# nickirk/pymes

Measured on AMD Instinct MI355X. Metric: ccsd_iteration_time, lower is better.
Workload: dtype f64

## Files before the change

### pymes_amd/csrc/kernels.hip

```cpp
#include <hip/hip_runtime.h>
#include <type_traits>

#include <algorithm>
#include <atomic>
#include <chrono>
#include <cmath>
#include <cstdio>
#include <cstdlib>
#include <cstring>
#include <mutex>
#include <stdexcept>
#include <string>
#include <vector>

#include "device_api.h"
#include "diis_small.h"

#define HIP_CHECK(expr)                                                                   \
    do {                                                                                  \
        hipError_t err__ = (expr);                                                        \
        if (err__ != hipSuccess)                                                          \
            throw std::runtime_error(std::string("HIP error: ") + hipGetErrorString(err__) + \
                                     " at " __FILE__ ":" + std::to_string(__LINE__));     \
    } while (0)
// ... 1476 lines not shown
                for (int j = 0; j < NN; ++j) acc[i][j] = fma(p.x[i][e], p.y[j][e], acc[i][j]);
    __shared__ double sh[4][MM * NN];
    const int lane = threadIdx.x & 63, w = threadIdx.x >> 6;
#pragma unroll
    for (int i = 0; i < MM; ++i)
#pragma unroll
        for (int j = 0; j < NN; ++j) {
            const double s = wave_sum(acc[i][j]);
            if (lane == 0) sh[w][i * NN + j] = s;
        }
    __syncthreads();
    if (threadIdx.x < MM * NN)
        partial[(long)blockIdx.x * (MM * NN) + threadIdx.x] =
            (sh[0][threadIdx.x] + sh[1][threadIdx.x]) + (sh[2][threadIdx.x] + sh[3][threadIdx.x]);
}
__global__ void __launch_bounds__(256) gram_stage2_kernel(const double* __restrict__ partial, int nblocks, int cnt,
                                                          double* __restrict__ out) {
    __shared__ double sh[4];
    const int idx = blockIdx.x;
    double s = 0.0;
    for (int b = threadIdx.x; b < nblocks; b += blockDim.x) s += partial[(long)b * cnt + idx];
    s = block_sum(s, sh);
    if (threadIdx.x == 0) out[idx] = s;
}

template <int MM, int NN>
struct LinMulti {
    const double* x[MM];
    double* y[NN];
    double c[MM][NN];
    double beta[NN];
};
template <int MM, int NN, int VEC>
__global__ void __launch_bounds__(256) lincomb_multi_kernel(const LinMulti<MM, NN> p, int n, long len) {
    typedef double vec_t __attribute__((ext_vector_type(VEC)));
    const long nvec = len / VEC;
    for (long e = blockIdx.x * 256L + threadIdx.x; e < nvec; e += (long)gridDim.x * 256L) {
        vec_t xv[MM], out[NN];
#pragma unroll
        for (int i = 0; i < MM; ++i) xv[i] = reinterpret_cast<const vec_t*>(p.x[i])[e];
#pragma unroll
        for (int j = 0; j < NN; ++j) {
            vec_t s = 0.0;
            if (j < n && p.beta[j] != 0.0) s = p.beta[j] * reinterpret_cast<const vec_t*>(p.y[j])[e];
            out[j] = s;
        }
#pragma unroll
        for (int i = 0; i < MM; ++i)
#pragma unroll
            for (int j = 0; j < NN; ++j) out[j] += p.c[i][j] * xv[i];
#pragma unroll
        for (int j = 0; j < NN; ++j)
            if (j < n) reinterpret_cast<vec_t*>(p.y[j])[e] = out[j];
    }
    if (VEC > 1 && blockIdx.x == 0 && threadIdx.x == 0)
        for (long e = nvec * VEC; e < len; ++e) {
            double xs[MM], out[NN];
#pragma unroll
            for (int i = 0; i < MM; ++i) xs[i] = p.x[i][e];
#pragma unroll
            for (int j = 0; j < NN; ++j) out[j] = (j < n && p.beta[j] != 0.0) ? p.beta[j] * p.y[j][e] : 0.0;
#pragma unroll
            for (int i = 0; i < MM; ++i)
#pragma unroll
                for (int j = 0; j < NN; ++j) out[j] += p.c[i][j] * xs[i];
#pragma unroll
            for (int j = 0; j < NN; ++j)
                if (j < n) p.y[j][e] = out[j];
        }
}

__global__ void cmul_kernel(const double* __restrict__ mr, const double* __restrict__ mi, const double* xr, const double* xi,
                            double* yr, double* yi, long n) {
    for (long e = blockIdx.x * (long)blockDim.x + threadIdx.x; e < n; e += (long)gridDim.x * blockDim.x) {
        const double a = xr[e], b = xi[e], c = mr[e], d = mi[e];
        yr[e] = c * a - d * b;
        yi[e] = c * b + d * a;
    }
}

__global__ void exchange_split_kernel(const double* __restrict__ u, double* __restrict__ us, double* __restrict__ w,
                                      double* __restrict__ dg, int no, int nv, long total) {
    const long o = no, v = nv;
    for (long e = blockIdx.x * (long)blockDim.x + threadIdx.x; e < total; e += (long)gridDim.x * blockDim.x) {
        const long j = e % o, i = (e / o) % o, b = (e / (o * o)) % v, a = e / (o * o * v);
        const double x = u[e], y = u[((b * v + a) * o + j) * o + i];
        const double ua = 0.5 * (x - y);
        us[e] = 0.5 * (x + y);
        w[e] = i > j ? ua : (i < j ? -ua : 0.0);
        if (i == j) dg[(a * v + b) * o + i] = ua;
    }
}
__global__ void sgn_ij_add_kernel(double* __restrict__ D, const double* __restrict__ R, int no, long total) {
    const long o = no;
    for (long e = blockIdx.x * (long)blockDim.x + threadIdx.x; e < total; e += (long)gridDim.x * blockDim.x) {
        const long j = e % o, i = (e / o) % o;
        if (i != j) D[e] += (i > j ? R[e] : -R[e]);
    }
}

struct EomDiagWs {
    long S1, Sa, Si, A2, a_, i_, IJ, AJ, AB, Z1, X1, total;
    __host__ __device__ EomDiagWs(long o, long v) {
        long p = 0;
        S1 = p; p += v * o;  Sa = p; p += v;  Si = p; p += o;  A2 = p; p += v * o;  a_ = p; p += v;  i_ = p; p += o;
        IJ = p; p += o * o;  AJ = p; p += v * o;  AB = p; p += v * v;  Z1 = p; p += v * o * o;  X1 = p; p += v * v * o;
        total = p;
    }
};
__global__ void __launch_bounds__(256) eom_diag_sums_kernel(const double* __restrict__ V, const double* __restrict__ T,
                                                            double* __restrict__ ws, int no, int nv) {
    __shared__ double sh[4];
    const long o = no, v = nv;
    const EomDiagWs w(o, v);
    auto Vx = [&](long k, long l, long c, long d) { return V[((k * o + l) * v + c) * v + d]; };
    auto Tx = [&](long a, long b, long i, long j) { return T[((a * v + b) * o + i) * o + j]; };
    const long e = blockIdx.x;
    const int t = threadIdx.x;
    double s = 0.0;
    if (e < w.Sa) {
        const long a = e / o, i = e % o;
        for (long x = t; x < o * v; x += 256) {
            const long j = x / v, b = x % v;
            s += (2.0 * Vx(j, i, b, a) - Vx(j, i, a, b)) * (2.0 * Tx(b, a, j, i) - Tx(a, b, j, i));
        }
    } else if (e < w.Si) {
        const long a = e - w.Sa;
        for (long x = t; x < o * o * v; x += 256) {
            const long j = x / (o * v), k = (x / v) % o, b = x % v;
            s += (2.0 * Vx(j, k, b, a) - Vx(j, k, a, b)) * Tx(a, b, j, k);
        }
    } else if (e < w.A2) {
        const long i = e - w.Si;
        for (long x = t; x < o * v * v; x += 256) {
            const long j = x / (v * v), c = (x / v) % v, b = x % v;
            s += Vx(j, i, c, b) * Tx(b, c, j, i);
        }
    } else if (e < w.a_) {
        const long a = (e - w.A2) / o, i = (e - w.A2) % o;
        for (long x = t; x < o * v; x += 256) {
            const long k = x / v, c = x % v;
            const double tca = Tx(c, a, k, i), tac = Tx(a, c, k, i);
            s += (2.0 * Vx(k, i, c, a) - 2.0 * Vx(k, i, a, c)) * tca + (Vx(k, i, a, c) - 2.0 * Vx(k, i, c, a)) * tac;
            double vb = 0.0;
            for (long b = 0; b < v; ++b) vb += Vx(k, i, c, b);
            s += vb * tac;
        }
    } else if (e < w.i_) {
        const long a = e - w.a_;
        for (long x = t; x < o * o * v; x += 256) {
            const long k = x / (o * v), l = (x / v) % o, c = x % v;
            s += Vx(k, l, c, a) * (Tx(a, c, k, l) - 2.0 * Tx(c, a, k, l));
        }
    } else if (e < w.IJ) {
        const long i = e - w.i_;
        for (long x = t; x < o * v * v; x += 256) {
            const long k = x / (v * v), c = (x / v) % v, d = x % v;
            s += (Vx(k, i, d, c) - 2.0 * Vx(k, i, c, d)) * Tx(c, d, k, i);
        }
    } else if (e < w.AJ) {
        const long i = (e - w.IJ) / o, j = (e - w.IJ) % o;
        for (long x = t; x < v * v; x += 256) {
            const long c = x / v, d = x % v;
            s += Vx(i, j, c, d) * Tx(c, d, i, j);
        }
    } else if (e < w.AB) {
        const long a = (e - w.AJ) / o, j = (e - w.AJ) % o;
        for (long x = t; x < o * v; x += 256) {
            const long k = x / v, c = x % v;
            s += Vx(k, j, a, c) * Tx(a, c, k, j);
        }
    } else if (e < w.Z1) {
        const long a = (e - w.AB) / v, b = (e - w.AB) % v;
        for (long x = t; x < o * o; x += 256) {
            const long k = x / o, l = x % o;
            s += Vx(k, l, a, b) * Tx(a, b, k, l);
        }
    } else if (e < w.X1) {
        const long r = e - w.Z1, a = r / (o * o), i = (r / o) % o, j = r % o;
        for (long x = t; x < o * v; x += 256) {
            const long k = x / v, c = x % v;
            s += Vx(k, j, a, c) * Tx(c, a, k, i);
        }
    } else {
        const long r = e - w.X1, a = r / (v * o), b = (r / o) % v, j = r % o;
        for (long k = t; k < o; k += 256) s += Vx(k, j, a, b) * Tx(a, b, k, j);
    }
    s = block_sum(s, sh);
    if (t == 0) ws[e] = s;
}
__global__ void eom_diag_singles_kernel(const double* __restrict__ ws, const double* __restrict__ dai, const double* __restrict__ iaai,
                                        const double* __restrict__ iaia, double* __restrict__ d1, int no, int nv) {
    const long o = no, v = nv;
    const EomDiagWs w(o, v);
    const long e = blockIdx.x * (long)blockDim.x + threadIdx.x;
    if (e >= v * o) return;
    const long a = e / o, i = e % o;
    d1[e] = dai[e] + 2.0 * iaai[e] - iaia[e] + ws[w.S1 + e] - ws[w.Sa + a] - ws[w.Si + i];
}
__global__ void __launch_bounds__(256) eom_diag_doubles_kernel(const double* __restrict__ V, const double* __restrict__ T,
                                                               const double* __restrict__ ws, const double* __restrict__ dai,
                                                               const double* __restrict__ iaai, const double* __restrict__ iaia,
                                                               const double* __restrict__ ijij, const double* __restrict__ abab,
                                                               double* __restrict__ d2, int no, int nv, long total) {
    const long o = no, v = nv;
    const EomDiagWs w(o, v);
    auto Vx = [&](long k, long l, long c, long d) { return V[((k * o + l) * v + c) * v + d]; };
    auto Tx = [&](long a, long b, long i, long j) { return T[((a * v + b) * o + i) * o + j]; };
    auto half = [&](long a, long b, long i, long j) {
        const long ai = a * o + i;
        double r = dai[ai] + iaai[ai] - 2.0 * iaia[ai] + ws[w.A2 + ai] + ws[w.a_ + a] + ws[w.i_ + i] -
                   2.0 * ws[w.X1 + (a * v + b) * o + j] - 2.0 * ws[w.IJ + i * o + j] + ws[w.Z1 + (a * o + i) * o + j] +
                   ws[w.AJ + a * o + j];
        double y = 0.0;
        for (long k = 0; k < o; ++k) y += Vx(k, i, a, b) * Tx(a, b, k, j);
        for (long c = 0; c < v; ++c) y += Vx(i, j, c, a) * Tx(c, b, i, j);
        return r + y;
    };
    for (long e = blockIdx.x * (long)blockDim.x + threadIdx.x; e < total; e += (long)gridDim.x * blockDim.x) {
        const long j = e % o, i = (e / o) % o, b = (e / (o * o)) % v, a = e / (o * o * v);
        d2[e] = half(a, b, i, j) + half(b, a, j, i) + ijij[i * o + j] + ws[w.IJ + i * o + j] + ws[w.AB + a * v + b] + abab[a * v + b];
    }
}
__global__ void cshift_inv_kernel(const double* __restrict__ d, double zr, double zi, double hr, double hi, double shift,
                                  double* __restrict__ mr, double* __restrict__ mi, long n) {
    for (long e = blockIdx.x * (long)blockDim.x + threadIdx.x; e < n; e += (long)gridDim.x * blockDim.x) {
        const double x = zr - hr * d[e] + shift, y = zi - hi * d[e];
        const double q = x * x + y * y;
        mr[e] = x / q;
        mi[e] = -y / q;
    }
}

struct TauK {
    double* tau; const double* t2; const double* t1;
    long total;
    int no, nv;
};
__device__ __forceinline__ void tau_body(const TauK& k, const unsigned vb, const unsigned vgrid) {
    double* __restrict__ tau = k.tau;
    const double* __restrict__ t2 = k.t2;
    const double* __restrict__ t1 = k.t1;
    const int no = k.no, nv = k.nv;
    const long total = k.total;
    for (long idx = vb * (long)blockDim.x + threadIdx.x; idx < total; idx += (long)vgrid * blockDim.x) {
        long r = idx;
        const int j = (int)(r % no); r /= no;
        const int i = (int)(r % no); r /= no;
        const int b = (int)(r % nv);
        const int a = (int)(r / nv);
        tau[idx] = t2[idx] + t1[a * no + i] * t1[b * no + j];
    }
}
__global__ void tau_kernel(const TauK k) { tau_body(k, blockIdx.x, gridDim.x); }

__device__ __forceinline__ void unrank_pair(long r, int& x, int& y) {
    long xx = (long)((sqrt(8.0 * (double)r + 1.0) - 1.0) * 0.5);
    while (xx * (xx + 1) / 2 > r) --xx;
    while ((xx + 1) * (xx + 2) / 2 <= r) ++xx;
    x = (int)xx;
    y = (int)(r - xx * (xx + 1) / 2);
}

__global__ void __launch_bounds__(256) ladder_pack_V_kernel(const double* __restrict__ V, double* __restrict__ Vp,
                                                            double* __restrict__ Vm, int nr, int nv, long rp0,
                                                            int nt, long ntp, long npp, long npm) {
    __shared__ double sA[32][33], sB[32][33];
    const long bid = blockIdx.x;
    const long row = bid / ntp;
    const long tp = bid - row * ntp;
    int a = 1, b = 0, tc, td;
    if (nr > 0) unrank_pair(rp0 + row, a, b);
    unrank_pair(tp, tc, td);
    const double* __restrict__ Vab = V + (nr > 0 ? (long)a * nr + b : rp0 + row) * nv * nv;
    const int tx = threadIdx.x & 31, ty = threadIdx.x >> 5;
    const int c0 = tc * 32, d0 = td * 32;
#pragma unroll
    for (int j = 0; j < 4; ++j) {
        const int y = ty + 8 * j;
        if (c0 + y < nv && d0 + tx < nv) sA[y][tx] = Vab[(long)(c0 + y) * nv + d0 + tx];
        if (d0 + y < nv && c0 + tx < nv) sB[y][tx] = Vab[(long)(d0 + y) * nv + c0 + tx];
    }
    __syncthreads();
#pragma unroll
    for (int j = 0; j < 4; ++j) {
        const int y = ty + 8 * j;
        const int c = c0 + y, d = d0 + tx;
        if (c < nv && d < nv && c >= d) {
            const double x1 = sA[y][tx], x2 = sB[tx][y];
            Vp[row * npp + (long)c * (c + 1) / 2 + d] = x1 + x2;
            if (c > d) Vm[row * npm + (long)c * (c - 1) / 2 + d] = (a > b) ? x1 - x2 : 0.0;
        }
    }
}

__global__ void ladder_dress_tfrag_kernel(const double* __restrict__ t1, double* __restrict__ tf, int no, int nv, int nk, long total) {
    const long e = blockIdx.x * (long)blockDim.x + threadIdx.x;
    if (e >= total) return;
    const int L = (int)(e & 63), kk = (int)((e >> 6) % nk), tile = (int)((e >> 6) / nk);
    const int a = 16 * tile + (L & 15), k = 4 * kk + (L >> 4);
    tf[e] = (a < nv && k < no) ? -t1[(long)a * no + k] : 0.0;
}

template <int NK>
__global__ void __launch_bounds__(64) ladder_dress_kernel(const double* __restrict__ V, const double* __restrict__ Pk,
                                                          const double* __restrict__ tf, double* __restrict__ W, int no,
                                                          int nv, long ld, long row0, long row1, double sgn, long ntp) {
    constexpr int TP = 16 * 16 + 16;
    __shared__ double turn[16 * TP];
    const int lane = threadIdx.x, g = lane >> 4, c = lane & 15;
    const long idx = blockIdx.x >> 3;
    const long cdb = (blockIdx.x & 7) + 8 * (idx / ntp), tp = idx % ntp;
    if (cdb * 16 >= ld) return;
    int ta_, tb_;
    unrank_pair(tp, ta_, tb_);
    const int a0 = ta_ * 16, b0 = tb_ * 16;
    const long tri0 = (long)a0 * (a0 + 1) / 2;
    if (tri0 + (long)15 * a0 + 120 + b0 + 15 < row0 || tri0 + b0 >= row1) return;
    double ta[NK], tb[NK];
#pragma unroll
    for (int kk = 0; kk < NK; ++kk) {
        ta[kk] = tf[((long)ta_ * NK + kk) * 64 + lane];
        tb[kk] = tf[((long)tb_ * NK + kk) * 64 + lane];
    }
    typedef unsigned v2u __attribute__((ext_vector_type(2)));
    constexpr unsigned kOff = 0x80000000u;
    const long col = cdb * 16 + c;
    const unsigned lo = (unsigned)(8 * ((long)g * ld + col));
    const unsigned lo_last = (unsigned)(8 * ((long)(min(4 * (NK - 1) + g, no - 1) - 4 * (NK - 1)) * ld + col));
    const unsigned ldb = (unsigned)(8 * ld);
    const __amdgpu_buffer_rsrc_t rPa = __builtin_amdgcn_make_buffer_rsrc(const_cast<double*>(Pk + (long)a0 * no * ld), 0, kOff, 0x00020000);
    const __amdgpu_buffer_rsrc_t rPb = __builtin_amdgcn_make_buffer_rsrc(const_cast<double*>(Pk + (long)b0 * no * ld), 0, kOff, 0x00020000);
    const __amdgpu_buffer_rsrc_t rV = __builtin_amdgcn_make_buffer_rsrc(const_cast<double*>(V + (tri0 - row0) * ld), 0, kOff, 0x00020000);
    const __amdgpu_buffer_rsrc_t rW = __builtin_amdgcn_make_buffer_rsrc(W + (tri0 - row0) * ld, 0, kOff, 0x00020000);
    unsigned vo[4];
#pragma unroll
    for (int r = 0; r < 4; ++r) {
        const long a = a0 + g + 4 * r;
        vo[r] = a < nv ? (unsigned)(8 * ((a * (a + 1) / 2 - tri0) * ld + col)) : kOff;
    }
    auto row_off = [&](int r, int x) {
        const int a = a0 + g + 4 * r;
        const long row = (long)a * (a + 1) / 2 + x;
        return (x <= a && row >= row0 && row < row1) ? vo[r] : kOff;
    };
    constexpr int PA = 1, NBP = 2 * (PA + 1), VA = 3, NBV = 2 * (VA + 1);
    double pf[NBP][NK], vin[NBV][4];
    auto fetch_p = [&](int n) {
        const int x0 = n < 16 ? a0 : b0, i = n < 16 ? n : n - 16;
        const unsigned so = (unsigned)(min(x0 + i, nv - 1) - x0) * (unsigned)no * ldb;
        const __amdgpu_buffer_rsrc_t rs = n < 16 ? rPa : rPb;
#pragma unroll
        for (int kk = 0; kk < NK - 1; ++kk)
            pf[n % NBP][kk] = __builtin_bit_cast(double, __builtin_amdgcn_raw_buffer_load_b64(rs, lo, so + 4u * kk * ldb, 0));
        pf[n % NBP][NK - 1] = __builtin_bit_cast(double, __builtin_amdgcn_raw_buffer_load_b64(rs, lo_last, so + 4u * (NK - 1) * ldb, 0));
    };
    auto fetch_v = [&](int n) {
        const int x = b0 + n - 16;
#pragma unroll
        for (int r = 0; r < 4; ++r)
            vin[n % NBV][r] = __builtin_bit_cast(double, __builtin_amdgcn_raw_buffer_load_b64(rV, row_off(r, x), (unsigned)x * ldb, 2));
    };
#pragma unroll
    for (int n = 0; n < 2 * PA; ++n) fetch_p(n);
#pragma unroll
    for (int p = 0; p < 8; ++p) {
        const int n0 = 2 * p, n1 = n0 + 1;
        fetch_p(n0 + 2 * PA);
        fetch_p(n1 + 2 * PA);
        if (n0 + 2 * VA >= 16) { fetch_v(n0 + 2 * VA); fetch_v(n1 + 2 * VA); }
        v4d acc0 = {0.0, 0.0, 0.0, 0.0}, acc1 = {0.0, 0.0, 0.0, 0.0};
#pragma unroll
        for (int kk = 0; kk < NK; ++kk) {
            acc0 = __builtin_amdgcn_mfma_f64_16x16x4f64(tb[kk], pf[n0 % NBP][kk], acc0, 0, 0, 0);
            acc1 = __builtin_amdgcn_mfma_f64_16x16x4f64(tb[kk], pf[n1 % NBP][kk], acc1, 0, 0, 0);
        }
#pragma unroll
        for (int rb = 0; rb < 4; ++rb) {
            turn[n0 * TP + (g + 4 * rb) * 16 + c] = acc0[rb];
            turn[n1 * TP + (g + 4 * rb) * 16 + c] = acc1[rb];
        }
    }
    __builtin_amdgcn_fence(__ATOMIC_SEQ_CST, "wavefront");
    __builtin_amdgcn_wave_barrier();
    const double s2 = sgn > 0.0 ? -1.0 : 1.0;
#pragma unroll
    for (int p = 0; p < 8; ++p) {
        const int b = 2 * p, n0 = 16 + b, n1 = n0 + 1;
        if (n0 + 2 * PA < 32) { fetch_p(n0 + 2 * PA); fetch_p(n1 + 2 * PA); }
        if (n0 + 2 * VA < 32) { fetch_v(n0 + 2 * VA); fetch_v(n1 + 2 * VA); }
        v4d acc0, acc1;
#pragma unroll
        for (int r = 0; r < 4; ++r) {
            acc0[r] = fma(s2, turn[(g + 4 * r) * TP + b * 16 + c], vin[n0 % NBV][r]);
            acc1[r] = fma(s2, turn[(g + 4 * r) * TP + (b + 1) * 16 + c], vin[n1 % NBV][r]);
        }
#pragma unroll
        for (int kk = 0; kk < NK; ++kk) {
            acc0 = __builtin_amdgcn_mfma_f64_16x16x4f64(ta[kk], pf[n0 % NBP][kk], acc0, 0, 0, 0);
            acc1 = __builtin_amdgcn_mfma_f64_16x16x4f64(ta[kk], pf[n1 % NBP][kk], acc1, 0, 0, 0);
        }
#pragma unroll
        for (int h = 0; h < 2; ++h) {
            const int bb = b0 + b + h;
#pragma unroll
            for (int r = 0; r < 4; ++r) {
                const double val = (sgn > 0.0 && a0 + g + 4 * r == bb) ? 0.0 : (double)(h ? acc1[r] : acc0[r]);
                __builtin_amdgcn_raw_buffer_store_b64(__builtin_bit_cast(v2u, val), rW, row_off(r, bb), (unsigned)bb * ldb, 2);
            }
        }
    }
}

struct PackTK {
    const double* T; const double* t1; double* Sp; double* Am;
    long ldp, ldm, rp0;
    int no, nv, flags;
};
__device__ __forceinline__ void ladder_pack_T_body(const PackTK& k, const unsigned vb) {
    const double* __restrict__ T = k.T;
    const double* __restrict__ t1 = k.t1;
    double* __restrict__ Sp = k.Sp;
    double* __restrict__ Am = k.Am;
    const int no = k.no, nv = k.nv, flags = k.flags;
    const long ldp = k.ldp, ldm = k.ldm;
    const long row = k.rp0 + vb;
    int c, d;
    unrank_pair(row, c, d);
    const bool row_half = flags & dev::PACK_ROW_HALF, prow = flags & dev::PACK_AM_PROWS,
               col_half = flags & dev::PACK_COL_HALF, pcol = flags & dev::PACK_AM_PCOLS;
    const long o2 = (long)no * no;
    const double* __restrict__ T1 = T ? T + ((long)c * nv + d) * o2 : nullptr;
    const double* __restrict__ T2 = T ? T + ((long)d * nv + c) * o2 : nullptr;
    const double fr = (c == d && row_half) ? 0.25 : 0.5;
    const long mrow = prow ? row : (long)c * (c - 1) / 2 + d;
    const bool has_m = prow || c > d;
    if (threadIdx.x == 0) {
        const long opp = (long)no * (no + 1) / 2, mcols = pcol ? opp : opp - no;
        if (ldp > opp) Sp[row * ldp + opp] = 0.0;
        if (has_m && ldm > mcols) Am[mrow * ldm + mcols] = 0.0;
    }
    for (int e = threadIdx.x; e < o2; e += blockDim.x) {
        const int i = e / no, j = e - i * no;
        if (i < j) continue;
        double x1 = 0.0, x2 = 0.0;
        if (T) { x1 = T1[e]; x2 = T2[e]; }
        if (t1) {
            x1 += t1[(long)c * no + i] * t1[(long)d * no + j];
            x2 += t1[(long)d * no + i] * t1[(long)c * no + j];
        }
        Sp[row * ldp + (long)i * (i + 1) / 2 + j] = ((i == j && col_half) ? 0.5 * fr : fr) * (x1 + x2);
        if (has_m && (pcol || i > j)) {
            const long mcol = pcol ? (long)i * (i + 1) / 2 + j : (long)i * (i - 1) / 2 + j;
            Am[mrow * ldm + mcol] = (c > d && i > j) ? 0.5 * (x1 - x2) : 0.0;
        }
    }
}
__global__ void ladder_pack_T_kernel(const PackTK k) { ladder_pack_T_body(k, blockIdx.x); }

struct UnpackK {
    const double* L; double* R;
    double beta;
    long total;
    int no, nv;
};
__device__ __forceinline__ void ladder_unpack_body(const UnpackK& k, const unsigned vb, const unsigned vgrid) {
    const double* __restrict__ L = k.L;
    double* __restrict__ R = k.R;
    const double beta = k.beta;
    const int no = k.no, nv = k.nv;
    const long total = k.total;
    const long opp = (long)no * (no + 1) / 2, ld = (long)no * no;
    for (long idx = vb * (long)blockDim.x + threadIdx.x; idx < total; idx += (long)vgrid * blockDim.x) {
        long r = idx;
        const int j = (int)(r % no); r /= no;
        const int i = (int)(r % no); r /= no;
        const int b = (int)(r % nv);
        const int a = (int)(r / nv);
        const int ah = max(a, b), al = min(a, b), ih = max(i, j), il = min(i, j);
        const double* __restrict__ row = L + ((long)ah * (ah + 1) / 2 + al) * ld;
        double v = row[(long)ih * (ih + 1) / 2 + il];
        if (a != b && i != j) {
            const double x = row[opp + (long)ih * (ih - 1) / 2 + il];
            v += ((a > b) == (i > j)) ? x : -x;
        }
        R[idx] = (beta != 0.0) ? beta * R[idx] + v : v;
    }
}
__global__ void ladder_unpack_kernel(const UnpackK k) { ladder_unpack_body(k, blockIdx.x, gridDim.x); }

struct RingOpK {
    const double* Wd; const double* Ud; double* M; double* N1;
    double a1, a2;
    int no, nv;
};
__device__ __forceinline__ void ring_operands_body(const RingOpK& q, const unsigned vb) {
    const double* __restrict__ Wd = q.Wd;
    const double* __restrict__ Ud = q.Ud;
    double* __restrict__ M = q.M;
    double* __restrict__ N1 = q.N1;
    const double a1 = q.a1, a2 = q.a2;
    const int no = q.no, nv = q.nv;
    extern __shared__ double tile[];
    constexpr int CT = 32;
    const int k = vb / nv, b = vb - k * nv;
    const long ov = (long)no * nv;
    const double* __restrict__ wd = Wd + ((long)k * nv + b) * ((long)nv * no);
    const double* __restrict__ ud = Ud + ((long)k * nv + b) * ((long)no * nv);
    const long col = (long)b * no;
    for (int c0 = 0; c0 < nv; c0 += CT) {
        const int nc = min(CT, nv - c0);
        for (int e = threadIdx.x; e < no * CT; e += blockDim.x) {
            const int j = e / CT, cc = e - j * CT;
            if (cc < nc) tile[j * (CT + 1) + cc] = ud[(long)j * nv + c0 + cc];
        }
        __syncthreads();
        for (int e = threadIdx.x; e < nc * no; e += blockDim.x) {
            const int cc = e / no, j = e - cc * no;
            const double u = tile[j * (CT + 1) + cc];
            const double w = wd[(long)(c0 + cc) * no + j];
            const long off = ((long)(c0 + cc) * no + k) * ov + col + j;
            N1[off] = -u;
            M[off] = a1 * w - a2 * u;
        }
        __syncthreads();
    }
}
__global__ void __launch_bounds__(256) ring_operands_kernel(const RingOpK q) { ring_operands_body(q, blockIdx.x); }

struct LayoutsK {
    const double* T; double* Td; double* Tx; double* Ttd;
    double ca, cb;
    int no, nv;
};
template <bool RESIDUAL>
__device__ __forceinline__ void t2_layouts_body(const LayoutsK& k, const unsigned vb) {
    const double* __restrict__ T = k.T;
    double* __restrict__ Td = k.Td;
    double* __restrict__ Tx = k.Tx;
    double* __restrict__ Ttd = k.Ttd;
    const int no = k.no, nv = k.nv;
    const double ca = k.ca, cb = k.cb;
    extern __shared__ double tile[];
    const int a = vb / nv, b = vb - a * nv;
    const long o2 = (long)no * no, ov = (long)no * nv;
    const double* __restrict__ Tab = T + ((long)a * nv + b) * o2;
    const double* __restrict__ Tba = T + ((long)b * nv + a) * o2;
    const long base = (long)a * no * ov + (long)b * no;
    for (int e = threadIdx.x; e < o2; e += blockDim.x) {
        const int i = e / no, j = e - i * no;
        const double x = Tab[e];
        tile[i * (no + 1) + j] = x;
        const long off = base + (long)i * ov + j;
        if (Td) Td[off] = x;
        Ttd[off] = RESIDUAL ? 2.0 * x - Tba[e] : ca * x + cb * Tba[e];
    }
    __syncthreads();
    for (int e = threadIdx.x; e < o2; e += blockDim.x) {
        const int j = e / no, i = e - j * no;
        Tx[base + (long)j * ov + i] = tile[i * (no + 1) + j];
    }
}
template <bool RESIDUAL>
__global__ void __launch_bounds__(256) t2_layouts_kernel(const LayoutsK k) { t2_layouts_body<RESIDUAL>(k, blockIdx.x); }

struct AssembleK {
    const double* V; const double* L; const double* N; const double* D; const double* X; double* R;
    double xd;
    int no, nv;
};
__device__ __forceinline__ void residual_assemble_body(const AssembleK& k, const unsigned vb) {
    const double* V = k.V;
    const double* __restrict__ L = k.L;
    const double* __restrict__ N = k.N;
    const double* __restrict__ D = k.D;
    const double* __restrict__ X = k.X;
    double* R = k.R;
    const int no = k.no, nv = k.nv;
    const double xd = k.xd;
    extern __shared__ double S[];
    int a, b;
    unrank_pair(vb, a, b);
    const int p = no + 1;
    const long o2 = (long)no * no, ov = (long)no * nv, opp = (long)no * (no + 1) / 2;
    const long ab = ((long)a * nv + b) * o2, ba = ((long)b * nv + a) * o2;
    const long tab = (long)a * no * ov + (long)b * no, tba = (long)b * no * ov + (long)a * no;
    for (int e = threadIdx.x; e < o2; e += blockDim.x) {
        const int i = e / no, j = e - i * no;
        double v = N[ab + e] + D[tab + (long)i * ov + j] + X[tba + (long)i * ov + j];
        if (xd != 0.0) v += xd * X[tab + (long)i * ov + j];
        S[i * p + j] = v;
    }
    __syncthreads();
    for (int e = threadIdx.x; e < o2; e += blockDim.x) {
        const int j = e / no, i = e - j * no;
        double v = N[ba + e] + D[tba + (long)j * ov + i] + X[tab + (long)j * ov + i];
        if (xd != 0.0) v += xd * X[tba + (long)j * ov + i];
        S[i * p + j] += v;
    }
    __syncthreads();
    const double* __restrict__ row = L ? L + ((long)a * (a + 1) / 2 + b) * o2 : nullptr;
    for (int e = threadIdx.x; e < o2; e += blockDim.x) {
        const int i = e / no, j = e - i * no;
        const int ih = max(i, j), il = min(i, j);
        double ls = 0.0, la = 0.0;
        if (row) {
            ls = row[(long)ih * (ih + 1) / 2 + il];
            if (a != b && i != j) la = row[opp + (long)ih * (ih - 1) / 2 + il];
        }
        const double sgn = i > j ? 1.0 : -1.0;
        R[ab + e] = (V ? V[ab + e] : 0.0) + ls + sgn * la + S[i * p + j];
        if (a != b) R[ba + e] = (V ? V[ba + e] : 0.0) + ls - sgn * la + S[j * p + i];
    }
}
__global__ void __launch_bounds__(256) residual_assemble_kernel(const AssembleK k) { residual_assemble_body(k, blockIdx.x); }

__global__ void __launch_bounds__(256) energy_norms_pairs_kernel(const double* __restrict__ f, const double* __restrict__ t1,
                                                                 const double* __restrict__ tc, const double* __restrict__ Edir,
                                                                 const double* __restrict__ Eex, const double* __restrict__ dtc,
                                                                 int no, int nv, long r0, long npairs, int with_t1,
                                                                 double* __restrict__ partial) {
    __shared__ double sh[4];
    double s1 = 0.0, s2 = 0.0, s3 = 0.0, s4 = 0.0, s0 = 0.0, s5 = 0.0;
    const long o2 = (long)no * no;
    for (long tile = blockIdx.x; tile < 2 * npairs; tile += gridDim.x) {
        int a, b;
        unrank_pair(r0 + (tile >> 1), a, b);
        if (tile & 1) {
            if (a == b) continue;
            const int x = a; a = b; b = x;
        }
        const double* __restrict__ x = tc + tile * o2;
        const double* __restrict__ d = dtc ? dtc + tile * o2 : nullptr;
        const double* __restrict__ ed = Edir + ((long)a * nv + b) * o2;
        const double* __restrict__ ex = Eex + ((long)a * nv + b) * o2;
        for (int e = threadIdx.x; e < o2; e += blockDim.x) {
            const double v = x[e];
            double tau = v;
            if (t1) {
                const int i = e / no, j = e - i * no;
                tau += t1[a * no + i] * t1[b * no + j];
            }
            s1 += tau * ed[e];
            s2 += tau * ex[e];
            s3 += v * v;
            if (d) s4 += d[e] * d[e];
        }
    }
    if (with_t1 && t1 && f) {
        const long n = no + nv, ov = (long)no * nv;
        for (long e = blockIdx.x * (long)blockDim.x + threadIdx.x; e < ov; e += (long)gridDim.x * blockDim.x) {
            const long a = e / no, i = e - a * no;
            const double y = t1[e];
            s0 += f[i * n + no + a] * y;
            s5 += y * y;
        }
    }
    const double q0 = block_sum(s0, sh), q1 = block_sum(s1, sh), q2 = block_sum(s2, sh), q3 = block_sum(s3, sh),
                 q4 = block_sum(s4, sh), q5 = block_sum(s5, sh);
    if (threadIdx.x == 0) {
        partial[0 * kDotBlocks + blockIdx.x] = q0;
        partial[1 * kDotBlocks + blockIdx.x] = q1;
        partial[2 * kDotBlocks + blockIdx.x] = q2;
        partial[3 * kDotBlocks + blockIdx.x] = q3;
        partial[4 * kDotBlocks + blockIdx.x] = q4;
        partial[5 * kDotBlocks + blockIdx.x] = q5;
    }
}

__global__ void __launch_bounds__(256) pairs_pack_kernel(const double* __restrict__ full, double* __restrict__ Xc,
                                                         int no, int nv, long r0) {
    int a, b;
    unrank_pair(r0 + blockIdx.x, a, b);
    const long o2 = (long)no * no;
    const double* __restrict__ ab = full + ((long)a * nv + b) * o2;
    const double* __restrict__ ba = full + ((long)b * nv + a) * o2;
    double* __restrict__ out = Xc + (long)blockIdx.x * 2 * o2;
    for (int e = threadIdx.x; e < o2; e += blockDim.x) {
        out[e] = ab[e];
        out[o2 + e] = (a != b) ? ba[e] : 0.0;
    }
}
__global__ void __launch_bounds__(256) pairs_unpack_kernel(const double* __restrict__ Xc, double* __restrict__ full,
                                                           int no, int nv, long r0) {
    int a, b;
    unrank_pair(r0 + blockIdx.x, a, b);
    const long o2 = (long)no * no;
    const double* __restrict__ in = Xc + (long)blockIdx.x * 2 * o2;
    double* __restrict__ ab = full + ((long)a * nv + b) * o2;
    double* __restrict__ ba = full + ((long)b * nv + a) * o2;
    for (int e = threadIdx.x; e < o2; e += blockDim.x) {
        ab[e] = in[e];
        if (a != b) ba[e] = in[o2 + e];
    }
}
__global__ void __launch_bounds__(256) cc_update_pairs_kernel(double* __restrict__ tc, double* __restrict__ dtc,
                                                              const double* __restrict__ rc, const double* __restrict__ eo,
                                                              const double* __restrict__ ev, double shift, double delta,
                                                              int no, long r0) {
    int a, b;
    unrank_pair(r0 + blockIdx.x, a, b);
    const long o2 = (long)no * no, base = (long)blockIdx.x * 2 * o2;
    const double eab = ev[a] + ev[b];
    for (int e = threadIdx.x; e < 2 * o2; e += blockDim.x) {
        const int t = e >= o2 ? e - (int)o2 : e;
        const int i = t / no, j = t - i * no;
        const double x = rc[base + e] * (1.0 / (eo[i] + eo[j] - eab + shift));
        dtc[base + e] = x;
        tc[base + e] += delta * x;
    }
}
__global__ void __launch_bounds__(256) residual_assemble_pairs_kernel(const double* __restrict__ V, const double* __restrict__ L,
                                                                      const double* __restrict__ Np, const double* __restrict__ D,
                                                                      const double* __restrict__ X, double* __restrict__ Rc,
// ... 3084 lines not shown
```

Baseline: 0.1634.

## Split ladder dress kernel into interior and edge tile paths with V preloaded

Splits the ladder dressing kernel into a templated tile routine with a fast interior path that drops per-element bounds and row-range predicates, used when the tile is off-diagonal and fully inside the row window. The edge path skips whole MFMA pairs whose output rows fall outside the window. It also reorders the computation so V is loaded as the initial accumulator of the first MFMA stage, with the sign folded into tb, instead of added after the transposed turn. This is meant to cut address and predicate ALU work and wasted MFMAs on boundary tiles, at the cost of more code size and register pressure from two instantiations.

```diff
diff --git a/pymes_amd/csrc/kernels.hip b/pymes_amd/csrc/kernels.hip
--- a/pymes_amd/csrc/kernels.hip
+++ b/pymes_amd/csrc/kernels.hip
@@ -1802,114 +1802,165 @@
     tf[e] = (a < nv && k < no) ? -t1[(long)a * no + k] : 0.0;
 }
 
+typedef unsigned v2u_dress __attribute__((ext_vector_type(2)));
+
+template <int NK, bool EDGE>
+__device__ __forceinline__ void ladder_dress_tile(const double* __restrict__ V, const double* __restrict__ Pk,
+                                                  const double* __restrict__ tf, double* __restrict__ W, double* turn,
+                                                  int no, int nv, long ld, long row0, long row1, double sgn,
+                                                  int ta_, int tb_, long cdb) {
+    constexpr int TP = 16 * 16 + 16;
+    constexpr unsigned kOff = 0x80000000u;
+    const int lane = threadIdx.x, g = lane >> 4, c = lane & 15;
+    const int a0 = ta_ * 16, b0 = tb_ * 16;
+    const long tri0 = (long)a0 * (a0 + 1) / 2;
+    double ta[NK], tb[NK];
+#pragma unroll
+    for (int kk = 0; kk < NK; ++kk) {
+        ta[kk] = tf[((long)ta_ * NK + kk) * 64 + lane];
+        tb[kk] = tf[((long)tb_ * NK + kk) * 64 + lane];
+    }
+    if (sgn > 0.0) {
+#pragma unroll
+        for (int kk = 0; kk < NK; ++kk) tb[kk] = -tb[kk];
+    }
+    const long col = cdb * 16 + c;
+    const unsigned ldb = (unsigned)(8 * ld);
+    const unsigned lo = (unsigned)(8 * ((long)g * ld + col));
+    unsigned lk[NK];
+#pragma unroll
+    for (int kk = 0; kk < NK - 1; ++kk) lk[kk] = lo + 4u * kk * ldb;
+    lk[NK - 1] = (unsigned)(8 * ((long)min(4 * (NK - 1) + g, no - 1) * ld + col));
+    const __amdgpu_buffer_rsrc_t rPa = __builtin_amdgcn_make_buffer_rsrc(const_cast<double*>(Pk + (long)a0 * no * ld), 0, kOff, 0x00020000);
+    const __amdgpu_buffer_rsrc_t rPb = __builtin_amdgcn_make_buffer_rsrc(const_cast<double*>(Pk + (long)b0 * no * ld), 0, kOff, 0x00020000);
+    const __amdgpu_buffer_rsrc_t rV = __builtin_amdgcn_make_buffer_rsrc(const_cast<double*>(V + (tri0 - row0) * ld), 0, kOff, 0x00020000);
+    const __amdgpu_buffer_rsrc_t rW = __builtin_amdgcn_make_buffer_rsrc(W + (tri0 - row0) * ld, 0, kOff, 0x00020000);
+    unsigned vo[4];
+    int pr[4];
+#pragma unroll
+    for (int r = 0; r < 4; ++r) {
+        const int a = a0 + g + 4 * r;
+        pr[r] = (a - a0) * a0 + (a - a0) * (a - a0 + 1) / 2;
+        vo[r] = (!EDGE || a < nv) ? (unsigned)(8 * ((long)pr[r] * ld + col)) : kOff;
+    }
+    unsigned vl[4];
+#pragma unroll
+    for (int r = 0; r < 4; ++r) vl[r] = lo + 4u * r * ldb;
+    const int rlo = (int)max(-1L, min(row0 - tri0, 1L << 30)), rhi = (int)max(-1L, min(row1 - tri0, 1L << 30));
+    const unsigned span = (unsigned)max(0, rhi - rlo);
+    constexpr int PA = 1, NBP = 2 * (PA + 1), VA = 2, NBV = 2 * (VA + 1);
+    double pf[NBP][NK], vin[NBV][4];
+    auto fetch_p = [&](int n) {
+        const int x0 = n < 16 ? a0 : b0, i = n < 16 ? n : n - 16;
+        const unsigned so = (unsigned)(min(x0 + i, nv - 1) - x0) * (unsigned)no * ldb;
+        const __amdgpu_buffer_rsrc_t rs = n < 16 ? rPa : rPb;
+#pragma unroll
+        for (int kk = 0; kk < NK; ++kk)
+            pf[n % NBP][kk] = __builtin_bit_cast(double, __builtin_amdgcn_raw_buffer_load_b64(rs, lk[kk], so, 0));
+    };
+    auto fetch_v = [&](int n) {
+        const int a = a0 + n;
+        const unsigned so = ((unsigned)(n * a0 + b0) + (unsigned)(n * (n + 1) / 2)) * ldb;
+#pragma unroll
+        for (int r = 0; r < 4; ++r) {
+            unsigned off = vl[r];
+            if (EDGE) {
+                const int b = b0 + g + 4 * r, rel = n * a0 + n * (n + 1) / 2 + b;
+                if (!(a < nv && b <= a && (unsigned)(rel - rlo) < span)) off = kOff;
+            }
+            vin[n % NBV][r] = __builtin_bit_cast(double, __builtin_amdgcn_raw_buffer_load_b64(rV, off, so, 2));
+        }
+    };
+    auto live_a = [&](int n) {
+        const int a = a0 + n;
+        if (a >= nv || b0 > a) return false;
+        const int lo = n * a0 + n * (n + 1) / 2 + b0, hi = lo + min(15, a - b0);
+        return lo < rhi && hi >= rlo;
+    };
+    auto live_b = [&](int j) {
+        const int bb = b0 + j, d0 = max(a0, bb) - a0, d1 = min(a0 + 15, nv - 1) - a0;
+        if (d0 > d1) return false;
+        const int lo = d0 * a0 + d0 * (d0 + 1) / 2 + bb, hi = d1 * a0 + d1 * (d1 + 1) / 2 + bb;
+        return lo < rhi && hi >= rlo;
+    };
+#pragma unroll
+    for (int n = 0; n < 2 * PA; ++n) fetch_p(n);
+#pragma unroll
+    for (int n = 0; n < 2 * VA; ++n) fetch_v(n);
+#pragma unroll
+    for (int p = 0; p < 8; ++p) {
+        const int n0 = 2 * p, n1 = n0 + 1;
+        fetch_p(n0 + 2 * PA);
+        fetch_p(n1 + 2 * PA);
+        if (n0 + 2 * VA < 16) { fetch_v(n0 + 2 * VA); fetch_v(n1 + 2 * VA); }
+        if (EDGE && !live_a(n0) && !live_a(n1)) continue;
+        v4d acc0, acc1;
+#pragma unroll
+        for (int r = 0; r < 4; ++r) { acc0[r] = vin[n0 % NBV][r]; acc1[r] = vin[n1 % NBV][r]; }
+#pragma unroll
+        for (int kk = 0; kk < NK; ++kk) {
+            acc0 = __builtin_amdgcn_mfma_f64_16x16x4f64(tb[kk], pf[n0 % NBP][kk], acc0, 0, 0, 0);
+            acc1 = __builtin_amdgcn_mfma_f64_16x16x4f64(tb[kk], pf[n1 % NBP][kk], acc1, 0, 0, 0);
+        }
+#pragma unroll
+        for (int rb = 0; rb < 4; ++rb) {
+            turn[n0 * TP + (g + 4 * rb) * 16 + c] = acc0[rb];
+            turn[n1 * TP + (g + 4 * rb) * 16 + c] = acc1[rb];
+        }
+    }
+    __builtin_amdgcn_fence(__ATOMIC_SEQ_CST, "wavefront");
+    __builtin_amdgcn_wave_barrier();
+#pragma unroll
+    for (int p = 0; p < 8; ++p) {
+        const int b = 2 * p, n0 = 16 + b, n1 = n0 + 1;
+        if (n0 + 2 * PA < 32) { fetch_p(n0 + 2 * PA); fetch_p(n1 + 2 * PA); }
+        if (EDGE && !live_b(b) && !live_b(b + 1)) continue;
+        v4d acc0, acc1;
+#pragma unroll
+        for (int r = 0; r < 4; ++r) {
+            acc0[r] = turn[(g + 4 * r) * TP + b * 16 + c];
+            acc1[r] = turn[(g + 4 * r) * TP + (b + 1) * 16 + c];
+        }
+#pragma unroll
+        for (int kk = 0; kk < NK; ++kk) {
+            acc0 = __builtin_amdgcn_mfma_f64_16x16x4f64(ta[kk], pf[n0 % NBP][kk], acc0, 0, 0, 0);
+            acc1 = __builtin_amdgcn_mfma_f64_16x16x4f64(ta[kk], pf[n1 % NBP][kk], acc1, 0, 0, 0);
+        }
+#pragma unroll
+        for (int h = 0; h < 2; ++h) {
+            const int bb = b0 + b + h;
+#pragma unroll
+            for (int r = 0; r < 4; ++r) {
+                double val = h ? acc1[r] : acc0[r];
+                unsigned off = vo[r];
+                if (EDGE) {
+                    const int a = a0 + g + 4 * r;
+                    if (!(bb <= a && (unsigned)(pr[r] + bb - rlo) < span)) off = kOff;
+                    if (sgn > 0.0 && a == bb) val = 0.0;
+                }
+                __builtin_amdgcn_raw_buffer_store_b64(__builtin_bit_cast(v2u_dress, val), rW, off, (unsigned)bb * ldb, 2);
+            }
+        }
+    }
+}
+
 template <int NK>
 __global__ void __launch_bounds__(64) ladder_dress_kernel(const double* __restrict__ V, const double* __restrict__ Pk,
                                                           const double* __restrict__ tf, double* __restrict__ W, int no,
                                                           int nv, long ld, long row0, long row1, double sgn, long ntp) {
-    constexpr int TP = 16 * 16 + 16;
-    __shared__ double turn[16 * TP];
-    const int lane = threadIdx.x, g = lane >> 4, c = lane & 15;
+    __shared__ double turn[16 * (16 * 16 + 16)];
     const long idx = blockIdx.x >> 3;
     const long cdb = (blockIdx.x & 7) + 8 * (idx / ntp), tp = idx % ntp;
     if (cdb * 16 >= ld) return;
     int ta_, tb_;
     unrank_pair(tp, ta_, tb_);
     const int a0 = ta_ * 16, b0 = tb_ * 16;
-    const long tri0 = (long)a0 * (a0 + 1) / 2;
-    if (tri0 + (long)15 * a0 + 120 + b0 + 15 < row0 || tri0 + b0 >= row1) return;
-    double ta[NK], tb[NK];
-#pragma unroll
-    for (int kk = 0; kk < NK; ++kk) {
-        ta[kk] = tf[((long)ta_ * NK + kk) * 64 + lane];
-        tb[kk] = tf[((long)tb_ * NK + kk) * 64 + lane];
-    }
-    typedef unsigned v2u __attribute__((ext_vector_type(2)));
-    constexpr unsigned kOff = 0x80000000u;
-    const long col = cdb * 16 + c;
-    const unsigned lo = (unsigned)(8 * ((long)g * ld + col));
-    const unsigned lo_last = (unsigned)(8 * ((long)(min(4 * (NK - 1) + g, no - 1) - 4 * (NK - 1)) * ld + col));
-    const unsigned ldb = (unsigned)(8 * ld);
-    const __amdgpu_buffer_rsrc_t rPa = __builtin_amdgcn_make_buffer_rsrc(const_cast<double*>(Pk + (long)a0 * no * ld), 0, kOff, 0x00020000);
-    const __amdgpu_buffer_rsrc_t rPb = __builtin_amdgcn_make_buffer_rsrc(const_cast<double*>(Pk + (long)b0 * no * ld), 0, kOff, 0x00020000);
-    const __amdgpu_buffer_rsrc_t rV = __builtin_amdgcn_make_buffer_rsrc(const_cast<double*>(V + (tri0 - row0) * ld), 0, kOff, 0x00020000);
-    const __amdgpu_buffer_rsrc_t rW = __builtin_amdgcn_make_buffer_rsrc(W + (tri0 - row0) * ld, 0, kOff, 0x00020000);
-    unsigned vo[4];
-#pragma unroll
-    for (int r = 0; r < 4; ++r) {
-        const long a = a0 + g + 4 * r;
-        vo[r] = a < nv ? (unsigned)(8 * ((a * (a + 1) / 2 - tri0) * ld + col)) : kOff;
-    }
-    auto row_off = [&](int r, int x) {
-        const int a = a0 + g + 4 * r;
-        const long row = (long)a * (a + 1) / 2 + x;
-        return (x <= a && row >= row0 && row < row1) ? vo[r] : kOff;
-    };
-    constexpr int PA = 1, NBP = 2 * (PA + 1), VA = 3, NBV = 2 * (VA + 1);
-    double pf[NBP][NK], vin[NBV][4];
-    auto fetch_p = [&](int n) {
-        const int x0 = n < 16 ? a0 : b0, i = n < 16 ? n : n - 16;
-        const unsigned so = (unsigned)(min(x0 + i, nv - 1) - x0) * (unsigned)no * ldb;
-        const __amdgpu_buffer_rsrc_t rs = n < 16 ? rPa : rPb;
-#pragma unroll
-        for (int kk = 0; kk < NK - 1; ++kk)
-            pf[n % NBP][kk] = __builtin_bit_cast(double, __builtin_amdgcn_raw_buffer_load_b64(rs, lo, so + 4u * kk * ldb, 0));
-        pf[n % NBP][NK - 1] = __builtin_bit_cast(double, __builtin_amdgcn_raw_buffer_load_b64(rs, lo_last, so + 4u * (NK - 1) * ldb, 0));
-    };
-    auto fetch_v = [&](int n) {
-        const int x = b0 + n - 16;
-#pragma unroll
-        for (int r = 0; r < 4; ++r)
-            vin[n % NBV][r] = __builtin_bit_cast(double, __builtin_amdgcn_raw_buffer_load_b64(rV, row_off(r, x), (unsigned)x * ldb, 2));
-    };
-#pragma unroll
-    for (int n = 0; n < 2 * PA; ++n) fetch_p(n);
-#pragma unroll
-    for (int p = 0; p < 8; ++p) {
-        const int n0 = 2 * p, n1 = n0 + 1;
-        fetch_p(n0 + 2 * PA);
-        fetch_p(n1 + 2 * PA);
-        if (n0 + 2 * VA >= 16) { fetch_v(n0 + 2 * VA); fetch_v(n1 + 2 * VA); }
-        v4d acc0 = {0.0, 0.0, 0.0, 0.0}, acc1 = {0.0, 0.0, 0.0, 0.0};
-#pragma unroll
-        for (int kk = 0; kk < NK; ++kk) {
-            acc0 = __builtin_amdgcn_mfma_f64_16x16x4f64(tb[kk], pf[n0 % NBP][kk], acc0, 0, 0, 0);
-            acc1 = __builtin_amdgcn_mfma_f64_16x16x4f64(tb[kk], pf[n1 % NBP][kk], acc1, 0, 0, 0);
-        }
-#pragma unroll
-        for (int rb = 0; rb < 4; ++rb) {
-            turn[n0 * TP + (g + 4 * rb) * 16 + c] = acc0[rb];
-            turn[n1 * TP + (g + 4 * rb) * 16 + c] = acc1[rb];
-        }
-    }
-    __builtin_amdgcn_fence(__ATOMIC_SEQ_CST, "wavefront");
-    __builtin_amdgcn_wave_barrier();
-    const double s2 = sgn > 0.0 ? -1.0 : 1.0;
-#pragma unroll
-    for (int p = 0; p < 8; ++p) {
-        const int b = 2 * p, n0 = 16 + b, n1 = n0 + 1;
-        if (n0 + 2 * PA < 32) { fetch_p(n0 + 2 * PA); fetch_p(n1 + 2 * PA); }
-        if (n0 + 2 * VA < 32) { fetch_v(n0 + 2 * VA); fetch_v(n1 + 2 * VA); }
-        v4d acc0, acc1;
-#pragma unroll
-        for (int r = 0; r < 4; ++r) {
-            acc0[r] = fma(s2, turn[(g + 4 * r) * TP + b * 16 + c], vin[n0 % NBV][r]);
-            acc1[r] = fma(s2, turn[(g + 4 * r) * TP + (b + 1) * 16 + c], vin[n1 % NBV][r]);
-        }
-#pragma unroll
-        for (int kk = 0; kk < NK; ++kk) {
-            acc0 = __builtin_amdgcn_mfma_f64_16x16x4f64(ta[kk], pf[n0 % NBP][kk], acc0, 0, 0, 0);
-            acc1 = __builtin_amdgcn_mfma_f64_16x16x4f64(ta[kk], pf[n1 % NBP][kk], acc1, 0, 0, 0);
-        }
-#pragma unroll
-        for (int h = 0; h < 2; ++h) {
-            const int bb = b0 + b + h;
-#pragma unroll
-            for (int r = 0; r < 4; ++r) {
-                const double val = (sgn > 0.0 && a0 + g + 4 * r == bb) ? 0.0 : (double)(h ? acc1[r] : acc0[r]);
-                __builtin_amdgcn_raw_buffer_store_b64(__builtin_bit_cast(v2u, val), rW, row_off(r, bb), (unsigned)bb * ldb, 2);
-            }
-        }
-    }
+    const long tri0 = (long)a0 * (a0 + 1) / 2, last = tri0 + (long)15 * a0 + 120 + b0 + 15;
+    if (last < row0 || tri0 + b0 >= row1) return;
+    if (ta_ > tb_ && a0 + 16 <= nv && tri0 + b0 >= row0 && last < row1)
+        ladder_dress_tile<NK, false>(V, Pk, tf, W, turn, no, nv, ld, row0, row1, sgn, ta_, tb_, cdb);
+    else
+        ladder_dress_tile<NK, true>(V, Pk, tf, W, turn, no, nv, ld, row0, row1, sgn, ta_, tb_, cdb);
 }
 
 struct PackTK {
```

Result: no change. 0.1631, median of 6 (-0.2%).
